# zhong-yy/volpick

Measured on AMD Instinct MI355X. Metric: waveform-windows/sec, higher is better.
Workload: dtype f32 (exact 3xbf16 split products, fp32 accumulate)

## Files before the change

volpick_amd/csrc/conv_b3.h:

```cpp
#pragma once
#include "bf16.h"
#include "conv_lds.h"

namespace vp {

typedef __bf16 bf16x8_b3 __attribute__((ext_vector_type(8)));

template <int C>
struct B3Image {
  static constexpr int CS = C + 8;
  bf16_t* img;
  int ps, c0;
};

__device__ __forceinline__ void b3_split(const float v, unsigned short& h, unsigned short& m, unsigned short& l) {
  h = to_bf16(v);
  const float r1 = v - from_bf16(h);
  m = to_bf16(r1);
  l = to_bf16(r1 - from_bf16(m));
}
__device__ __forceinline__ void b3_store4(bf16_t* img, const int ps, const int cs, const int col, const int ch, const float (&v)[4]) {
  const unsigned h0 = pack_bf16x2(v[0], v[1]), h1 = pack_bf16x2(v[2], v[3]);
  const float r0 = v[0] - bf16_lo(h0), r1 = v[1] - bf16_hi(h0), r2 = v[2] - bf16_lo(h1), r3 = v[3] - bf16_hi(h1);
  const unsigned m0 = pack_bf16x2(r0, r1), m1 = pack_bf16x2(r2, r3);
// ... 245 lines not shown
template <int C, int NC>
__device__ void b3c_dump(const bf16_t* img, const int c0, const int L, float* dst, const long ls, const int tid, const int nth) {
  using Q = B3Chunk<C, NC>;
  for (int k = tid; k < C * L; k += nth) {
    const int c = k / L, t = k - c * L;
    const bf16_t* p = img + (c >> 3) * Q::CHS + (t + c0) * 8 + (c & 7);
    dst[c * ls + t] = from_bf16(p[0]) + (from_bf16(p[Q::PS]) + from_bf16(p[2 * Q::PS]));
  }
}
#ifndef B3_EXP
#define B3_EXP 0
#endif
template <int C, int NC>
__device__ __forceinline__ void b3c_store4(bf16_t* img, const int col, const int quad, const float (&v)[4]) {
  using Q = B3Chunk<C, NC>;
  if (B3_EXP & 16) {
    asm volatile("" ::"v"(v[0]), "v"(v[1]), "v"(v[2]), "v"(v[3]));
    return;
  }
  const unsigned h0 = pack_bf16x2(v[0], v[1]), h1 = pack_bf16x2(v[2], v[3]);
  const float r0 = v[0] - bf16_lo(h0), r1 = v[1] - bf16_hi(h0), r2 = v[2] - bf16_lo(h1), r3 = v[3] - bf16_hi(h1);
  const unsigned m0 = pack_bf16x2(r0, r1), m1 = pack_bf16x2(r2, r3);
  const unsigned l0 = pack_bf16x2(r0 - bf16_lo(m0), r1 - bf16_hi(m0)), l1 = pack_bf16x2(r2 - bf16_lo(m1), r3 - bf16_hi(m1));
  bf16_t* p = img + (quad >> 1) * Q::CHS + col * 8 + (quad & 1) * 4;
  if (B3_EXP & 32) p = img + (quad >> 1) * Q::CHS + ((col >> 5) * 16 + (threadIdx.x & 15)) * 4;
  if (B3_EXP & 4) {
    asm volatile("" ::"v"(h0), "v"(h1), "v"(m0), "v"(m1), "v"(l0), "v"(l1), "v"(p));
    return;
  }
  *reinterpret_cast<uint2*>(p) = make_uint2(h0, h1);
  *reinterpret_cast<uint2*>(p + Q::PS) = make_uint2(m0, m1);
  *reinterpret_cast<uint2*>(p + 2 * Q::PS) = make_uint2(l0, l1);
}
template <int C, int NC, int TAPS>
__device__ __forceinline__ const bf16_t* b3c_lane_ptr(const bf16_t* img, const int col0, const int lane) {
  using G = B3Steps<C, TAPS>;
  const int g = lane >> 4;
  return img + (G::ch_of_lane(g) / 8) * B3Chunk<C, NC>::CHS + (col0 + (lane & 15) + G::tap_of_lane(g)) * 8;
}
struct B3NoSlot {
  __device__ __forceinline__ void operator()(int) const {}
};
template <int C, int NC, int TAPS, int NB, class Finish, class Slot = B3NoSlot>
__device__ __forceinline__ void b3c_mac_tiles(const bf16_t* p, const uint4 (&a)[B3Steps<C, TAPS>::STEPS * 3], Finish finish, Slot slot = Slot()) {
  using G = B3Steps<C, TAPS>;
  using Q = B3Chunk<C, NC>;
  constexpr int STEPS = G::STEPS;
  constexpr int AHEAD = 2, NBUF = AHEAD + 1, PAIRS = STEPS * NB;
  uint4 b[NBUF][3];
  auto load_b = [&](const int i) {
    const int s = i % STEPS, j = i / STEPS;
    const int off = ((C >= 32 ? s / G::KS : s * G::TPK) + j * 16) * 8 + (C >= 32 ? (s % G::KS) * 4 * Q::CHS : 0);
#pragma unroll
    for (int pc = 0; pc < 3; ++pc) b[i % NBUF][pc] = *reinterpret_cast<const uint4*>(p + pc * Q::PS + off);
  };
#pragma unroll
  for (int i = 0; i < AHEAD && i < PAIRS; ++i) load_b(i);
  f32x4 prev = {0.f, 0.f, 0.f, 0.f};
#pragma unroll
  for (int j = 0; j < NB; ++j) {
    f32x4 acc = {0.f, 0.f, 0.f, 0.f};
    __builtin_amdgcn_sched_barrier(0);
    if (j > 0) finish(j - 1, prev);
#pragma unroll
    for (int s = 0; s < STEPS; ++s) {
      const int i = j * STEPS + s;
// ... 27 lines not shown
      for (int pc = 0; pc < 3; ++pc) b[i & 1][h][pc] = *reinterpret_cast<const uint4*>(p + pc * Q::PS + off);
    }
  };
  load_b(0);
  f32x4 prev0 = {0.f, 0.f, 0.f, 0.f}, prev1 = prev0;
#pragma unroll
  for (int jp = 0; jp < NB / 2; ++jp) {
    f32x4 acc0 = {0.f, 0.f, 0.f, 0.f}, acc1 = acc0;
    __builtin_amdgcn_sched_barrier(0);
    if (jp > 0) {
      finish(2 * jp - 2, prev0);
      finish(2 * jp - 1, prev1);
    }
#pragma unroll
    for (int s = 0; s < STEPS; ++s) {
      const int i = jp * STEPS + s;
      if (i + 1 < PAIRS) load_b(i + 1);
      slot(i);
      constexpr int WP[6] = {2, 1, 0, 1, 0, 0}, XP[6] = {0, 1, 2, 0, 1, 0};
#pragma unroll
      for (int t = 0; t < 6; ++t) {
        acc0 = __builtin_amdgcn_mfma_f32_16x16x32_bf16(__builtin_bit_cast(bf16x8_b3, a[s * 3 + WP[t]]),
                                                      __builtin_bit_cast(bf16x8_b3, b[i & 1][0][XP[t]]), acc0, 0, 0, 0);
        acc1 = __builtin_amdgcn_mfma_f32_16x16x32_bf16(__builtin_bit_cast(bf16x8_b3, a[s * 3 + WP[t]]),
                                                      __builtin_bit_cast(bf16x8_b3, b[i & 1][1][XP[t]]), acc1, 0, 0, 0);
      }
    }
    __builtin_amdgcn_sched_barrier(0);
    prev0 = acc0;
    prev1 = acc1;
  }
  finish(NB - 2, prev0);
  finish(NB - 1, prev1);
}

template <int C, int NC, int TAPS, int NB>
__device__ __forceinline__ void b3c_mac_tiles_acc(const bf16_t* p, const uint4 (&a)[B3Steps<C, TAPS>::STEPS * 3], f32x4 (&acc)[NB]) {
  using G = B3Steps<C, TAPS>;
  using Q = B3Chunk<C, NC>;
  constexpr int STEPS = G::STEPS;
  constexpr int AHEAD = 1, NBUF = AHEAD + 1, PAIRS = STEPS * NB;
  uint4 b[NBUF][3];
  auto load_b = [&](const int i) {
    const int s = i % STEPS, j = i / STEPS;
    const int off = ((C >= 32 ? s / G::KS : s * G::TPK) + j * 16) * 8 + (C >= 32 ? (s % G::KS) * 4 * Q::CHS : 0);
#pragma unroll
    for (int pc = 0; pc < 3; ++pc) b[i % NBUF][pc] = *reinterpret_cast<const uint4*>(p + pc * Q::PS + off);
  };
  load_b(0);
#pragma unroll
  for (int j = 0; j < NB; ++j) {
#pragma unroll
    for (int s = 0; s < STEPS; ++s) {
      const int i = j * STEPS + s;
      if (i + AHEAD < PAIRS) load_b(i + AHEAD);
      __builtin_amdgcn_sched_barrier(0);
      constexpr int WP[6] = {2, 1, 0, 1, 0, 0}, XP[6] = {0, 1, 2, 0, 1, 0};
#pragma unroll
      for (int t = 0; t < 6; ++t)
        acc[j] = __builtin_amdgcn_mfma_f32_16x16x32_bf16(__builtin_bit_cast(bf16x8_b3, a[s * 3 + WP[t]]),
                                                        __builtin_bit_cast(bf16x8_b3, b[i % NBUF][XP[t]]), acc[j], 0, 0, 0);
      __builtin_amdgcn_sched_barrier(0);
    }
  }
}

// ... 72 lines not shown
```

volpick_amd/csrc/eqt_dec03.hip:

```cpp
#include <type_traits>

#include "conv_b3.h"
#include "conv_lds.h"
#include "eqt_kernels.h"
#include "net.h"

namespace vp {

namespace {

constexpr int D03_NTH = 512, D03_WAVES = 8;
using D_0 = LdsLayer<16, 0, 64, 2, 3, 1, -1, 0, 3, 1>;
using D_1 = LdsLayer<64, 0, 64, 2, 3, 1, -1, 0, 6, 1>;
using D_2 = LdsLayer<64, 0, 32, 2, 3, 1, -1, 0, 6, 1>;
using D_3 = LdsLayer<32, 0, 32, 2, 5, 1, -2, 0, 6, 1>;
constexpr int L0 = 47, L1 = 94, L2 = 188, L3 = 375, L4 = 750;
constexpr int C0 = 48, C1 = 96, C2 = 192, C3 = 384;
constexpr int S0 = 80, S1 = 112, S2 = 208, S3 = 400, BI = 4;
static_assert(S0 >= BI + C0 + 1 && S1 >= BI + 2 * C0 + 1 && S1 >= BI + C1 + 1 && S2 >= BI + 2 * C1 + 1 && S2 >= BI + C2 + 1 &&
                  S3 >= BI + 2 * C2 + 2 && S3 >= BI + C3 + 2,
              "image widths");
static_assert(S0 % 32 == 16 && S1 % 32 == 16 && S2 % 32 == 16 && S3 % 32 == 16, "bank-conflict-free strides");
constexpr int OFF0 = 0, OFF1 = OFF0 + 16 * S0, OFF2 = OFF1 + 64 * S1, OFF3 = OFF2 + 64 * S2, D03_LDS_FLOATS = OFF3 + 32 * S3;
static_assert(D03_LDS_FLOATS * 4 <= 160 * 1024 && OFF1 % 4 == 0 && OFF2 % 4 == 0 && OFF3 % 4 == 0, "LDS budget");

constexpr int B3_X1_NC = 112, B3_X2_NC = 208;
using QX1 = B3Chunk<64, B3_X1_NC>;
using QX2 = B3Chunk<64, B3_X2_NC>;
constexpr int B3_X1_PS = QX1::PS, B3_X2_PS = QX2::PS;
static_assert(B3_X1_NC >= C1 + 3 && B3_X2_NC >= C2 + 3, "every column stages 1 / 2 read has a place");
constexpr int B3_OFF_X2 = 0, B3_OFF_R = 3 * B3_X2_PS * 2;
constexpr int B3_OFF_X0 = B3_OFF_R, B3_OFF_X1 = B3_OFF_X0 + 16 * S0 * 4, B3_OFF_X3 = B3_OFF_R;
constexpr int B3_X3_NC = 400, B3_X3_C0 = 2;
using QX3 = B3Chunk<32, B3_X3_NC>;
constexpr int B3_OFF_EDGE = B3_OFF_X3 + 3 * QX3::PS * 2;
constexpr int B3_LDS_BYTES = B3_OFF_EDGE + D03_WAVES * 64 * 4;
static_assert(B3_X3_NC >= C3 + 4 + 0 && B3_X3_NC >= L3 + B3_X3_C0, "every column stage 3 reads has a place");
static_assert(B3_OFF_X1 + 3 * B3_X1_PS * 2 <= B3_LDS_BYTES && B3_LDS_BYTES <= 160 * 1024 && B3_OFF_R % 16 == 0 && B3_OFF_X1 % 16 == 0,
              "LDS budget of the bf16-piece variant");

struct Dec03Args {
  const float* x;
  int ls_x;
  long ws_x;
  float* y;
  int ls_y;
  long ws_y;
  const float* af[4];
  const float* bs[4];
  long af_stride[4];
  const uint4* af3[3];
  long af3_stride[3];
  const float* edge_w;
  const float* edge_b;
  int B, n_rows;
  int even_split;
  unsigned long long* clk;
};
struct Dec03DumpArgs : Dec03Args {
  float* dbg[3];
  int dbg_ls[3];
  long dbg_ws[3];
};

template <int S>
struct RowStore {
  float* img;
  unsigned len;
  __device__ __forceinline__ void operator()(int co, int t, float v) const { img[co * S + t] = ((unsigned)t < len) ? v : 0.f; }
  __device__ __forceinline__ bool all_valid(int t0, int t1) const { return (unsigned)t1 < len; }
// ... 27 lines not shown
          *reinterpret_cast<float2*>(row + t) =
              make_float2(fmaxf(acc[j][rr] + biasv[rr], 0.f), fmaxf(acc[j][rr + 1] + biasv[rr + 1], 0.f));
      }
    }
  }
};

struct Stage0Pieces {
  static constexpr bool custom_block_epilogue = true;
  bf16_t* img;
  __device__ __forceinline__ void quad(const int co, const int t, const float (&v)[4]) const {
    const float z[4] = {t < L1 ? v[0] : 0.f, t < L1 ? v[1] : 0.f, t < L1 ? v[2] : 0.f, t < L1 ? v[3] : 0.f};
    b3c_store4<64, B3_X1_NC>(img, t + 1, co >> 2, z);
  }
  template <class L>
  __device__ __forceinline__ void block_epilogue(const f32x4 (&acc)[L::NB], const float (&biasv)[4], const int mt, const int colb,
                                                 const int g, const int n) const {
    static_assert(L::P == 2 && L::RELU == 1 && L::OUT_OFF == 0 && L::COUT == 64, "stage 0 of the decoder");
#pragma unroll
    for (int j = 0; j < L::NB; ++j) {
      float v[4];
#pragma unroll
      for (int r = 0; r < 4; ++r) v[r] = fmaxf(acc[j][r] + biasv[r], 0.f);
      this->quad((mt & 3) * 16 + 4 * g, 2 * (colb + j * 16 + n) + (mt >> 2), v);
    }
  }
};
struct ClipQuad {
  bf16_t* img;
  int hi;
  __device__ __forceinline__ void quad(const int co, const int t, const float (&v)[4]) const {
    if (t < hi) b3c_store4<32, B3_X3_NC>(img, t + B3_X3_C0, co >> 2, v);
  }
};

template <bool B3, bool DUMP = false>
__global__ __launch_bounds__(D03_NTH) void eqt_dec03_kernel(const std::conditional_t<DUMP, Dec03DumpArgs, Dec03Args> a) {
  static_assert(!DUMP || B3, "DUMP instances exist for the default form only");
  extern __shared__ float4 d03_lds_raw[];
  float* lds = reinterpret_cast<float*>(d03_lds_raw);
  if constexpr (B3) {
    char* base = reinterpret_cast<char*>(d03_lds_raw);
    int o_r = B3_OFF_R / 16;
    asm volatile("" : "+v"(o_r));
    float* X0 = reinterpret_cast<float*>(base + 16 * o_r);
    bf16_t* X3 = reinterpret_cast<bf16_t*>(base + 16 * o_r);
    float* EDGE = reinterpret_cast<float*>(base + B3_OFF_EDGE);
    bf16_t* const X1 = reinterpret_cast<bf16_t*>(base + B3_OFF_X1);
    bf16_t* const X2 = reinterpret_cast<bf16_t*>(base + B3_OFF_X2);
    const int tid = threadIdx.x, lane = tid & 63, g = lane >> 4;
    const int wave_u = __builtin_amdgcn_readfirstlane(tid >> 6);
    int row = blockIdx.x;
    if (row >= a.n_rows) return;
    for (int i = tid; i < B3_LDS_BYTES / 16; i += D03_NTH) d03_lds_raw[i] = make_float4(0.f, 0.f, 0.f, 0.f);
    float pre[3];
    auto request = [&](int r) {
      const float* src = a.x + (long)r * a.ws_x + HALO;
#pragma unroll
      for (int k = 0; k < 3; ++k) {
        const int idx = tid + k * D03_NTH, c = idx / S0, t = idx - c * S0 - BI;
        pre[k] = (idx < 16 * S0 && (unsigned)t < (unsigned)L0) ? src[(long)c * a.ls_x + t] : 0.f;
      }
    };
    auto park = [&]() {
#pragma unroll
      for (int k = 0; k < 3; ++k) {
// ... 18 lines not shown
#if D3_CLOCK
    unsigned long long* clk = (a.clk && (tid & 255) == 0 && blockIdx.x == 0) ? a.clk + (tid >> 8) * 128 : nullptr;
    int stamp = 0;
#define D3_STAMP() \
  if (clk && stamp < 120) clk[stamp++] = __builtin_readcyclecounter();
#else
#define D3_STAMP()
#endif
    while (true) {
      const int next = row + gridDim.x;
      const bool more = next < a.n_rows;
      const int nd = more ? next / a.B : d;
      D3_STAMP()
      park();
      __syncthreads();
      D3_STAMP()
      uint4 a1[B3Steps<64, 3>::STEPS * 3];
      b3_load_a<64, 3>(a.af3[0] + d * a.af3_stride[0], wave_u, lane, a1);
      {
        Stage0Pieces st{X1};
        b3c_zero_rest<64, B3_X1_NC>(X1, 1, 1 + 2 * C0, tid, D03_NTH);
        conv_lds_areg<D_0, S0, BI, S0, BI>(X0, X0, areg0, bias0, wave_u, C0, st, 0, 1, lane);
      }
      const int n = lane & 15;
      {
        const int ph = wave_u >> 2, co0 = (wave_u & 3) * 16 + 4 * g;
        float bias1[4];
#pragma unroll
        for (int r = 0; r < 4; ++r) bias1[r] = a.bs[1][d * 64 + co0 + r];
        D3_STAMP()
        __syncthreads();
        D3_STAMP()
        if constexpr (DUMP) b3c_dump<64, B3_X1_NC>(X1, 1, L1, a.dbg[0] + (long)row * a.dbg_ws[0] + HALO, a.dbg_ls[0], tid, D03_NTH);
        b3c_mac_tile_pairs<64, B3_X1_NC, 3, 6>(b3c_lane_ptr<64, B3_X1_NC, 3>(X1, 0, lane), a1, [&](const int j, const f32x4 acc) {
          const int t = 2 * (j * 16 + n) + ph;
          float v[4];
#pragma unroll
          for (int r = 0; r < 4; ++r) v[r] = t < L2 ? fmaxf(acc[r] + bias1[r], 0.f) : 0.f;
          b3c_store4<64, B3_X2_NC>(X2, t + 1, co0 >> 2, v);
        });
      }
      D3_STAMP()
      uint4 a2[B3Steps<64, 3>::STEPS * 3];
      b3_load_a<64, 3>(a.af3[1] + d * a.af3_stride[1], wave_u & 3, lane, a2);
      __syncthreads();
      D3_STAMP()
      if constexpr (DUMP) b3c_dump<64, B3_X2_NC>(X2, 1, L2, a.dbg[1] + (long)row * a.dbg_ws[1] + HALO, a.dbg_ls[1], tid, D03_NTH);
      float eb;
      {
        constexpr int PADC = B3_X3_C0 + (B3_X3_NC - L3 - B3_X3_C0);
        if (tid < PADC * 12) {
          const int k = tid % PADC, cp = tid / PADC;
          const int col = k < B3_X3_C0 ? k : L3 + k;
          *reinterpret_cast<uint4*>(X3 + (cp >> 2) * QX3::PS + (cp & 3) * QX3::CHS + col * 8) = make_uint4(0u, 0u, 0u, 0u);
        }
        constexpr int n0 = (L3 - 2 - 2) >> 1;
        struct F3 {
          float x, y, z;
        };
        F3 ew[8];
        eb = a.edge_b[d * 32 + (lane >> 1)];
        const F3* e = reinterpret_cast<const F3*>(a.edge_w + ((long)d * 64 * 64 + lane) * 3 + (long)(8 * wave_u) * 64 * 3);
        const ClipQuad st{X3, L3 - 2};
        {
          const int mt2 = wave_u & 3, ph = mt2 >> 1, co0 = (mt2 & 1) * 16 + 4 * g, colb = (wave_u >> 2) * 96;
          float bias2[4];
#pragma unroll
          for (int r = 0; r < 4; ++r) bias2[r] = a.bs[2][d * 32 + co0 + r];
          b3c_mac_tile_pairs<64, B3_X2_NC, 3, 6>(b3c_lane_ptr<64, B3_X2_NC, 3>(X2, colb, lane), a2, [&](const int j, const f32x4 acc) {
            float v[4];
#pragma unroll
            for (int r = 0; r < 4; ++r) v[r] = fmaxf(acc[r] + bias2[r], 0.f);
            st.quad(co0, 2 * (colb + j * 16 + n) + ph, v);
            if constexpr (DUMP) {
              const int t = 2 * (colb + j * 16 + n) + ph;
              if (t < L3 - 2) {
                float* p = a.dbg[2] + (long)row * a.dbg_ws[2] + HALO + (long)co0 * a.dbg_ls[2] + t;
#pragma unroll
                for (int r = 0; r < 4; ++r) p[(long)r * a.dbg_ls[2]] = v[r];
              }
            }
          }, [&](const int i) {
            if (i % 2 == 0 && i / 2 < 8) ew[i / 2] = e[(i / 2) * 64];
          });
        }
        D3_STAMP()
        float pacc = 0.f;
        {
          float xk[3][8];
#pragma unroll
          for (int k = 0; k < 3; ++k) {
            uint4 q[3];
#pragma unroll
            for (int pc = 0; pc < 3; ++pc) q[pc] = *reinterpret_cast<const uint4*>(X2 + pc * QX2::PS + wave_u * QX2::CHS + (n0 + 1 + k) * 8);
            const unsigned* qh = reinterpret_cast<const unsigned*>(&q[0]);
            const unsigned* qm = reinterpret_cast<const unsigned*>(&q[1]);
            const unsigned* ql = reinterpret_cast<const unsigned*>(&q[2]);
#pragma unroll
            for (int i = 0; i < 4; ++i) {
              xk[k][2 * i] = (bf16_lo(qh[i]) + bf16_lo(qm[i])) + bf16_lo(ql[i]);
              xk[k][2 * i + 1] = (bf16_hi(qh[i]) + bf16_hi(qm[i])) + bf16_hi(ql[i]);
            }
          }
#pragma unroll
          for (int u = 0; u < 8; ++u) {
            pacc = fmaf(ew[u].x, xk[0][u], pacc);
            pacc = fmaf(ew[u].y, xk[1][u], pacc);
            pacc = fmaf(ew[u].z, xk[2][u], pacc);
          }
        }
        EDGE[wave_u * 64 + lane] = pacc;
      }
      D3_STAMP()
      uint4 a3[B3Steps<32, 5>::STEPS * 3];
      float bias3[4];
      b3_load_a<32, 5>(a.af3[2] + d * a.af3_stride[2], mt23, lane, a3);
#pragma unroll
      for (int r = 0; r < 4; ++r) bias3[r] = a.bs[3][d * 32 + mt23 * 8 + 2 * g + (r >> 1)];
      request(more ? next : row);
      load_stage0(nd);
      __syncthreads();
      D3_STAMP()
      if (blk23 == 1) {
        float acc = eb;
#pragma unroll
        for (int w8 = 0; w8 < D03_WAVES; ++w8) acc += EDGE[w8 * 64 + lane];
        unsigned short h, m, l;
        b3_split(fmaxf(acc, 0.f), h, m, l);
        const int ch = lane >> 1;
        bf16_t* q = X3 + (ch >> 3) * QX3::CHS + (L3 - 2 + (lane & 1) + B3_X3_C0) * 8 + (ch & 7);
        q[0] = h, q[QX3::PS] = m, q[2 * QX3::PS] = l;
        if constexpr (DUMP) {
          if (wave_u == 4) a.dbg[2][(long)row * a.dbg_ws[2] + HALO + (long)ch * a.dbg_ls[2] + L3 - 2 + (lane & 1)] = fmaxf(acc, 0.f);
        }
      }
      {
        float* yrow = a.y + (long)row * a.ws_y + HALO + (long)(mt23 * 8 + 2 * g) * a.ls_y;
        asm volatile("" ::"v"(bias3[0]), "v"(bias3[1]), "v"(bias3[2]), "v"(bias3[3]));
        auto stage3 = [&](const int colb, auto nb_tag) {
          constexpr int NB = decltype(nb_tag)::value;
          b3c_mac_tiles<32, B3_X3_NC, 5, NB>(b3c_lane_ptr<32, B3_X3_NC, 5>(X3, colb, lane), a3, [&](const int j, const f32x4 acc) {
            const int t = 2 * (colb + j * 16 + (lane & 15));
            if (t < L4) {
              *reinterpret_cast<float2*>(yrow + t) = make_float2(fmaxf(acc[0] + bias3[0], 0.f), fmaxf(acc[1] + bias3[1], 0.f));
              *reinterpret_cast<float2*>(yrow + a.ls_y + t) = make_float2(fmaxf(acc[2] + bias3[2], 0.f), fmaxf(acc[3] + bias3[3], 0.f));
            }
          });
        };
        if (a.even_split) {
          stage3(blk23 * 96, std::integral_constant<int, 6>{});
          stage3((blk23 + 2) * 96, std::integral_constant<int, 6>{});
        } else if (blk23 == 0) {
          stage3(0, std::integral_constant<int, 7>{});
          stage3(112, std::integral_constant<int, 7>{});
        } else {
          stage3(224, std::integral_constant<int, 5>{});
          stage3(304, std::integral_constant<int, 5>{});
        }
      }
      D3_STAMP()
      if (!more) break;
      row = next;
      d = nd;
      __syncthreads();
    }
#undef D3_STAMP
    return;
  }
  int off1 = OFF1 / 4, off2 = OFF2 / 4, off3 = OFF3 / 4;
  asm volatile("" : "+v"(off1), "+v"(off2), "+v"(off3));
  float* X0 = lds + OFF0;
  float* X1 = lds + 4 * off1;
  float* X2 = lds + 4 * off2;
  float* X3 = lds + 4 * off3;
  const int tid = threadIdx.x, lane = tid & 63;
  const int wave_u = __builtin_amdgcn_readfirstlane(tid >> 6);
  int row = blockIdx.x;
  if (row >= a.n_rows) return;
// ... 165 lines not shown
```

volpick_amd/csrc/eqt_tail_b3.hip:

```cpp
#include <type_traits>

#include "conv_b3.h"
#include "eqt_kernels.h"
#include "net.h"

namespace vp {

namespace {

constexpr int T_OUT = 6000;
constexpr int T3_NTH = 512, T3_WAVES = 8;
constexpr int HSB = 81, OUT_QS = 16 * HSB, OUT_PS = 2 * OUT_QS;
constexpr int HT_N = 43;
template <int TW_>
struct T3 {
  static constexpr int TW = TW_;
  static constexpr int NB4O = 3, NB4Y = TW_ > 1200 ? 3 : 2, NB5 = 5, NB6 = 5;
  static constexpr int C4 = 2 * (NB4O + NB4Y) * 16, C5 = 4 * NB5 * 16, C6 = T3_WAVES * NB6 * 16;
  static constexpr int PARK_COLS = TW_ > 1200 ? 176 : 168;
  static constexpr int NC4 = 208, NC5 = (2 * C4 > C5 + 16 ? 2 * C4 : C5 + 16), NC6 = C6 + 16;
  static constexpr int BLOCKS = (TW_ + 15) / 16;
  using Q4 = B3Chunk<32, NC4>;
  using Q5 = B3Chunk<16, NC5>;
  using Q6 = B3Chunk<16, NC6>;
  static constexpr bool GUARD5 = 2 * C5 > NC6;
  static constexpr bool ZERO6 = (TW_ + 12) / 2 + 7 >= 2 * C5;
  static constexpr int R0_BYTES = 3 * Q6::PS * 2, R1_BYTES = 3 * OUT_PS * 8;
  static constexpr int A5_N = 2 * B3Steps<16, 5>::STEPS * 3 * 64, A6_N = B3Steps<16, 7>::STEPS * 3 * 64;
  static constexpr int OFF_R1 = R0_BYTES, OFF_HT = OFF_R1 + R1_BYTES, OFF_A5 = OFF_HT + 3 * HT_N * 16 + 48, OFF_A6 = OFF_A5 + A5_N * 16;
  static constexpr int LDS_BYTES = OFF_A6 + A6_N * 16;
  static_assert(OFF_A5 % 16 == 0, "16-byte fragments");
  static_assert(3 * Q4::PS * 2 <= R0_BYTES && 3 * Q5::PS * 2 <= R1_BYTES && LDS_BYTES <= 160 * 1024 && OFF_R1 % 16 == 0 && OFF_HT % 16 == 0,
                "LDS budget");
  static_assert(NC4 >= PARK_COLS && NC5 >= C5 + 6 && NC6 >= C6 + 8 && NC5 >= 2 * C4 && (GUARD5 || NC6 >= 2 * C5) && HSB % 2 == 1,
                "every column a stage reads or writes has a place");
  static_assert(TW % 8 == 0, "tile grid: 16-byte stores of the heads, whole stage-3 samples");
  static_assert(TW + 11 <= 2 * C6 && C6 / 8 <= HSB - 1 && (BLOCKS + 15) / 16 <= T3_WAVES, "stage 6 / heads");
  static_assert((TW + 12) / 2 + 7 < NC6 && (!ZERO6 || 2 * C5 % 2 == 0), "the padded taps of stage 6 stay inside its input image");
  static_assert(TW / 2 + 6 + 6 <= 2 * C5 && TW / 2 + 6 + 6 <= NC6 && TW / 4 + 6 + 5 <= 2 * C4 && TW / 8 + 6 + 4 <= PARK_COLS, "halo chain");
  static_assert(((((TW + 12) / 2 + 7) / 2 + 1 + 5) / 2 + 4) < PARK_COLS, "closure of the kept outputs under the padded taps");
  static_assert(PARK_COLS * 8 <= 3 * T3_NTH && PARK_COLS * 8 > 2 * T3_NTH, "three (four channels x one sample) items per thread");
  static constexpr double GROUPS = 4.0 * (NB4O + NB4Y) * 5 + 8.0 * NB5 * 3 + 8.0 * NB6 * 4 + 5.0 * 7;
};

struct Tail3Args {
  const float* x3;
  int ls3;
  long ws3;
  float* y;
  const uint4 *af4, *af5, *af6;
  long af4_stride, af5_stride, af6_stride;
  const float *bs4, *bs5, *bs6;
  const uint4* head_t;
  const float* head_b;
  const float* flags;
  int B, n_tiles;
  int t_lo, tiles_per_row;
  unsigned long long* clk;
};
struct Tail3DumpArgs : Tail3Args {
  float* dbg[4];
  int dbg_ls[4];
  long dbg_ws[4];
};

struct Tile3 {
  int d, win, t0;
};
template <int TW>
__device__ __forceinline__ Tile3 tile3_id(const int tile, const Tail3Args& a) {
  const int row = tile / a.tiles_per_row, j = tile - row * a.tiles_per_row;
  return Tile3{row / a.B, row, a.t_lo + j * TW};
}

__device__ __forceinline__ void t3_finish(const f32x4 acc, const float (&bias)[4], const bool in, float (&v)[4]) {
#pragma unroll
  for (int r = 0; r < 4; ++r) v[r] = in ? fmaxf(acc[r] + bias[r], 0.f) : 0.f;
}

template <int TW_, bool DUMP = false>
__global__ __launch_bounds__(T3_NTH) void eqt_tail3_kernel(const std::conditional_t<DUMP, Tail3DumpArgs, Tail3Args> a) {
  static_assert(!DUMP || TW_ == 1200, "DUMP instances exist for the 1200-sample tiling only");
  using K = T3<TW_>;
  using Q5 = typename K::Q5;
  using Q6 = typename K::Q6;
  constexpr int TW = K::TW, NB4O = K::NB4O, NB4Y = K::NB4Y, NB5 = K::NB5, NB6 = K::NB6, PARK_COLS = K::PARK_COLS, NC4 = K::NC4,
                NC5 = K::NC5, NC6 = K::NC6, C5 = K::C5, BLOCKS = K::BLOCKS, OFF_R1 = K::OFF_R1, OFF_HT = K::OFF_HT, OFF_A5 = K::OFF_A5, OFF_A6 = K::OFF_A6,
                A5_N = K::A5_N, A6_N = K::A6_N, T3_LDS_BYTES = K::LDS_BYTES;
  (void)sizeof(Q5), (void)sizeof(Q6);
  extern __shared__ uint4 t3_lds[];
  char* base = reinterpret_cast<char*>(t3_lds);
  bf16_t* IN4 = reinterpret_cast<bf16_t*>(base);
  bf16_t* IN6 = IN4;
  bf16_t* IN5 = reinterpret_cast<bf16_t*>(base + OFF_R1);
  uint2* OUT6 = reinterpret_cast<uint2*>(base + OFF_R1);
  uint4* HT = reinterpret_cast<uint4*>(base + OFF_HT);
  uint4* A5 = reinterpret_cast<uint4*>(base + OFF_A5);
  uint4* A6 = reinterpret_cast<uint4*>(base + OFF_A6);
  const int tid = threadIdx.x, lane = tid & 63, n = lane & 15, g = lane >> 4;
  const int w = __builtin_amdgcn_readfirstlane(tid >> 6);
  int tile = blockIdx.x;
  if (tile >= a.n_tiles) return;
  for (int i = tid; i < T3_LDS_BYTES / 16; i += T3_NTH) t3_lds[i] = make_uint4(0u, 0u, 0u, 0u);
  Tile3 id = tile3_id<TW>(tile, a);
  unsigned long long* clk = (a.clk && tid == 0 && (int)blockIdx.x < a.B) ? a.clk + (long)blockIdx.x * 32 : nullptr;
  int n_done = 0;
  auto dump = [&](const int i, const int co, const int s, const int lo, const int len, const float (&v)[4]) {
    if constexpr (DUMP) {
      if ((unsigned)(s - lo) < (unsigned)len) {
        float* p = a.dbg[i] + (long)id.win * a.dbg_ws[i] + HALO + (long)co * a.dbg_ls[i] + s;
// ... 39 lines not shown

  uint4 a4[B3Steps<32, 5>::STEPS * 3];
  float bias4[4], bias5[4], bias6[4], bh;
  auto load_weights = [&](const int d) {
    b3_load_a<32, 5>(a.af4 + d * a.af4_stride, w & 1, lane, a4);
    for (int i = tid; i < A5_N; i += T3_NTH) A5[i] = a.af5[d * a.af5_stride + i];
    for (int i = tid; i < A6_N; i += T3_NTH) A6[i] = a.af6[d * a.af6_stride + i];
#pragma unroll
    for (int r = 0; r < 4; ++r) {
      bias4[r] = a.bs4[d * 16 + 4 * g + r];
      bias5[r] = a.bs5[d * 16 + 4 * g + r];
      bias6[r] = a.bs6[d * 8 + 4 * (g & 1) + r];
    }
    bh = a.head_b[d];
    if (tid < 3 * HT_N) HT[tid] = a.head_t[d * 3 * HT_N + tid];
  };
  __syncthreads();
  load_weights(id.d);

  while (true) {
    const int next = tile + gridDim.x;
    const bool more = next < a.n_tiles;
    const Tile3 nid = more ? tile3_id<TW>(next, a) : id;
    const int t0 = id.t0;
    const float win_flag = a.flags ? a.flags[id.win - id.d * a.B] : 0.f;
    T3_STAMP(0)
    park();
    __syncthreads();
    T3_STAMP(1)
    {
      const bool older = w < 4;
      const int ph = w & 1, colb = older ? (w >> 1) * (NB4O * 16) : 2 * NB4O * 16 + ((w - 4) >> 1) * (NB4Y * 16);
      const int lo = 6 - t0 / 4;
      auto finish = [&](const int j, const f32x4 acc) {
        const int t = 2 * (colb + j * 16 + n) + ph;
        float v[4];
        t3_finish(acc, bias4, (unsigned)(t - lo) < 1500u, v);
        b3c_store4<16, NC5>(IN5, t, g, v);
        if constexpr (DUMP) dump(0, 4 * g, t0 / 4 - 6 + t, t0 / 4, TW / 4, v);
      };
      if (older) b3c_mac_tiles<32, NC4, 5, NB4O>(b3c_lane_ptr<32, NC4, 5>(IN4, colb, lane), a4, finish);
      else b3c_mac_tiles<32, NC4, 5, NB4Y>(b3c_lane_ptr<32, NC4, 5>(IN4, colb, lane), a4, finish);
    }
    __syncthreads();
    T3_STAMP(2)
    {
      const int ph = w & 1, colb = (w >> 1) * (NB5 * 16);
      uint4 a5[B3Steps<16, 5>::STEPS * 3];
#pragma unroll
      for (int i = 0; i < B3Steps<16, 5>::STEPS * 3; ++i) a5[i] = A5[ph * (A5_N / 2) + i * 64 + lane];
      const int lo = 6 - t0 / 2;
      auto finish = [&](const int j, const f32x4 acc) {
        const int t = 2 * (colb + j * 16 + n) + ph;
        float v[4];
        t3_finish(acc, bias5, (unsigned)(t - lo) < 3000u, v);
        if (!K::GUARD5 || t < NC6) b3c_store4<16, NC6>(IN6, t, g, v);
        if constexpr (DUMP) dump(1, 4 * g, t0 / 2 - 6 + t, t0 / 2, TW / 2, v);
      };
      if (K::ZERO6) {
        constexpr int ZC = NC6 - 2 * C5, UNITS = 3 * 2 * ZC;
        for (int i = tid; i < UNITS; i += T3_NTH) {
          const int plane = i / ZC, col = 2 * C5 + (i - plane * ZC);
          *reinterpret_cast<uint4*>(IN6 + (plane >> 1) * Q6::PS + (plane & 1) * Q6::CHS + col * 8) = make_uint4(0u, 0u, 0u, 0u);
        }
      }
      b3c_mac_tiles<16, NC5, 5, NB5>(b3c_lane_ptr<16, NC5, 5>(IN5, colb + 1, lane), a5, finish);
    }
    __syncthreads();
    T3_STAMP(3)
    {
      const int colb = w * (NB6 * 16), ph = g >> 1;
      uint4 a6[B3Steps<16, 7>::STEPS * 3];
#pragma unroll
      for (int i = 0; i < B3Steps<16, 7>::STEPS * 3; ++i) a6[i] = A6[i * 64 + lane];
      const int lo = 6 - t0;
      uint2* q = OUT6 + (g & 1) * OUT_QS + ((2 * n + ph) & 15) * HSB + (n >> 3) + colb / 8;
      auto finish = [&](const int j, const f32x4 acc) {
        const int t = 2 * (colb + j * 16 + n) + ph;
        float v[4];
        t3_finish(acc, bias6, (unsigned)(t - lo) < (unsigned)T_OUT, v);
        if constexpr (DUMP) dump(2, 4 * (g & 1), t0 - 6 + t, t0, TW, v);
        if (B3_EXP & 16) {
          asm volatile("" ::"v"(v[0]), "v"(v[1]), "v"(v[2]), "v"(v[3]));
          return;
        }
        const unsigned h0 = pack_bf16x2(v[0], v[1]), h1 = pack_bf16x2(v[2], v[3]);
        const float r0 = v[0] - bf16_lo(h0), r1 = v[1] - bf16_hi(h0), r2 = v[2] - bf16_lo(h1), r3 = v[3] - bf16_hi(h1);
        const unsigned m0 = pack_bf16x2(r0, r1), m1 = pack_bf16x2(r2, r3);
        const unsigned l0 = pack_bf16x2(r0 - bf16_lo(m0), r1 - bf16_hi(m0)), l1 = pack_bf16x2(r2 - bf16_lo(m1), r3 - bf16_hi(m1));
        if (B3_EXP & 4) {
          asm volatile("" ::"v"(h0), "v"(h1), "v"(m0), "v"(m1), "v"(l0), "v"(l1), "v"(q));
          return;
        }
        q[2 * j] = make_uint2(h0, h1);
        q[2 * j + OUT_PS] = make_uint2(m0, m1);
        q[2 * j + 2 * OUT_PS] = make_uint2(l0, l1);
      };
      b3c_mac_tiles<16, NC6, 7, NB6>(b3c_lane_ptr<16, NC6, 7>(IN6, colb, lane), a6, finish, [&](const int i) {
        if (i < 12) request_part(nid, i);
      });
    }
    __syncthreads();
    T3_STAMP(4)
    if (w < (BLOCKS + 15) / 16) {
      f32x4 acc = {bh, bh, bh, bh};
      const uint2* bp = OUT6 + (16 * w + n);
      const uint4* ap = HT + (g - n + 15);
      constexpr int HD = 1, HB = HD + 1;
      uint4 av[HB][3], bv[HB][3];
      auto load_ab = [&](const int s, uint4 (&aa)[3], uint4 (&bb)[3]) {
        const int e = 4 * s + g + 1, chunk = (e & 15) * HSB + (e >> 4);
#pragma unroll
        for (int pc = 0; pc < 3; ++pc) {
          aa[pc] = ap[pc * HT_N + 4 * s];
          const uint2 c0 = bp[pc * OUT_PS + chunk], c1 = bp[pc * OUT_PS + OUT_QS + chunk];
          bb[pc] = make_uint4(c0.x, c0.y, c1.x, c1.y);
        }
      };
#pragma unroll
      for (int s = 0; s < HD && s < 7; ++s) load_ab(s, av[s % HB], bv[s % HB]);
#pragma unroll
      for (int s = 0; s < 7; ++s) {
        if (s + HD < 7) load_ab(s + HD, av[(s + HD) % HB], bv[(s + HD) % HB]);
        __builtin_amdgcn_sched_barrier(0);
        constexpr int WP[6] = {2, 1, 0, 1, 0, 0}, XP[6] = {0, 1, 2, 0, 1, 0};
#pragma unroll
        for (int t = 0; t < 6; ++t)
          acc = __builtin_amdgcn_mfma_f32_16x16x32_bf16(__builtin_bit_cast(bf16x8_b3, av[s % HB][WP[t]]),
                                                       __builtin_bit_cast(bf16x8_b3, bv[s % HB][XP[t]]), acc, 0, 0, 0);
        __builtin_amdgcn_sched_barrier(0);
      }
// ... 125 lines not shown
```

Measured before the change: 3.464 million.

## Slice 3xbf16 epilogue across K-steps and overlap weight reads with barriers

Splits each tile's epilogue (bias/relu, then hi/mid/lo bf16 split and store) into three parts. Each part runs during one of the next tile's K-steps, with sched_group_barrier interleaving MFMAs and the VALU/LDS work, so the epilogue hides under matrix math instead of stalling after each tile. In the tail kernel, the next stage's weight fragments are read from LDS before a custom s_waitcnt+s_barrier that leaves those reads outstanding. Store addresses are precomputed once per stage. This raises register pressure and makes correctness depend on hand-written waitcnt counts and on schedule hints.

After: 3.455 million, median of 2. Within noise of the previous version (-0.3%).

```diff
diff --git a/volpick_amd/csrc/conv_b3.h b/volpick_amd/csrc/conv_b3.h
--- a/volpick_amd/csrc/conv_b3.h
+++ b/volpick_amd/csrc/conv_b3.h
@@ -301,6 +301,60 @@
   *reinterpret_cast<uint2*>(p + Q::PS) = make_uint2(m0, m1);
   *reinterpret_cast<uint2*>(p + 2 * Q::PS) = make_uint2(l0, l1);
 }
+#ifndef B3C_SLICED
+#define B3C_SLICED 1
+#endif
+struct B3cSplit {
+  float v[4];
+  unsigned p0, p1;
+};
+template <int C, int NC>
+__device__ __forceinline__ bf16_t* b3c_quad_ptr(bf16_t* img, const int col, const int quad) {
+  using Q = B3Chunk<C, NC>;
+  if (B3_EXP & 32) return img + (quad >> 1) * Q::CHS + ((col >> 5) * 16 + (threadIdx.x & 15)) * 4;
+  return img + (quad >> 1) * Q::CHS + col * 8 + (quad & 1) * 4;
+}
+template <int C, int NC>
+__device__ __forceinline__ void b3c_store_piece(bf16_t* p, const int pc, const unsigned d0, const unsigned d1) {
+  if (B3_EXP & 4) {
+    asm volatile("" ::"v"(d0), "v"(d1), "v"(p));
+    return;
+  }
+  *reinterpret_cast<uint2*>(p + pc * B3Chunk<C, NC>::PS) = make_uint2(d0, d1);
+}
+template <class Values, class Store>
+struct B3cFinish {
+  using State = B3cSplit;
+  Values values;
+  Store store;
+  __device__ __forceinline__ void a(const int j, const f32x4 acc, State& s) const {
+    values(j, acc, s.v);
+    if (B3_EXP & 16) {
+      asm volatile("" ::"v"(s.v[0]), "v"(s.v[1]), "v"(s.v[2]), "v"(s.v[3]));
+      return;
+    }
+    s.p0 = pack_bf16x2(s.v[0], s.v[1]), s.p1 = pack_bf16x2(s.v[2], s.v[3]);
+    store(j, 0, s.p0, s.p1);
+  }
+  __device__ __forceinline__ void b(const int j, State& s) const {
+    if (B3_EXP & 16) return;
+    s.v[0] -= bf16_lo(s.p0), s.v[1] -= bf16_hi(s.p0), s.v[2] -= bf16_lo(s.p1), s.v[3] -= bf16_hi(s.p1);
+    s.p0 = pack_bf16x2(s.v[0], s.v[1]), s.p1 = pack_bf16x2(s.v[2], s.v[3]);
+    store(j, 1, s.p0, s.p1);
+  }
+  __device__ __forceinline__ void c(const int j, State& s) const {
+    if (B3_EXP & 16) return;
+    store(j, 2, pack_bf16x2(s.v[0] - bf16_lo(s.p0), s.v[1] - bf16_hi(s.p0)), pack_bf16x2(s.v[2] - bf16_lo(s.p1), s.v[3] - bf16_hi(s.p1)));
+  }
+  __device__ __forceinline__ void operator()(const int j, const f32x4 acc) const {
+    State s;
+    a(j, acc, s), b(j, s), c(j, s);
+  }
+};
+template <class Values, class Store>
+__device__ __forceinline__ B3cFinish<Values, Store> b3c_finish(Values values, Store store) {
+  return B3cFinish<Values, Store>{values, store};
+}
 template <int C, int NC, int TAPS>
 __device__ __forceinline__ const bf16_t* b3c_lane_ptr(const bf16_t* img, const int col0, const int lane) {
   using G = B3Steps<C, TAPS>;
@@ -394,6 +448,127 @@
   }
   finish(NB - 2, prev0);
   finish(NB - 1, prev1);
+}
+
+template <int MFMAS, int PER>
+__device__ __forceinline__ void b3c_spread() {
+#pragma unroll
+  for (int t = 0; t < MFMAS; ++t) {
+    __builtin_amdgcn_sched_group_barrier(0x008, 1, 0);
+    __builtin_amdgcn_sched_group_barrier(0x002 | 0x200, PER, 0);
+  }
+}
+template <int C, int NC, int TAPS, int NB, class Fin, class Slot = B3NoSlot>
+__device__ __forceinline__ void b3c_mac_tiles_sliced(const bf16_t* p, const uint4 (&a)[B3Steps<C, TAPS>::STEPS * 3], Fin fin, Slot slot = Slot()) {
+#if !B3C_SLICED
+  b3c_mac_tiles<C, NC, TAPS, NB>(p, a, fin, slot);
+#else
+  using G = B3Steps<C, TAPS>;
+  using Q = B3Chunk<C, NC>;
+  constexpr int STEPS = G::STEPS;
+  static_assert(STEPS >= 3, "three parts need three K-steps");
+  constexpr int AHEAD = 1, NBUF = AHEAD + 1, PAIRS = STEPS * NB;
+  uint4 b[NBUF][3];
+  auto load_b = [&](const int i) {
+    const int s = i % STEPS, j = i / STEPS;
+    const int off = ((C >= 32 ? s / G::KS : s * G::TPK) + j * 16) * 8 + (C >= 32 ? (s % G::KS) * 4 * Q::CHS : 0);
+#pragma unroll
+    for (int pc = 0; pc < 3; ++pc) b[i % NBUF][pc] = *reinterpret_cast<const uint4*>(p + pc * Q::PS + off);
+  };
+#pragma unroll
+  for (int i = 0; i < AHEAD && i < PAIRS; ++i) load_b(i);
+  f32x4 prev = {0.f, 0.f, 0.f, 0.f};
+  typename Fin::State st;
+#pragma unroll
+  for (int j = 0; j < NB; ++j) {
+    f32x4 acc = {0.f, 0.f, 0.f, 0.f};
+#pragma unroll
+    for (int s = 0; s < STEPS; ++s) {
+      const int i = j * STEPS + s;
+      __builtin_amdgcn_sched_barrier(0);
+      if (i + AHEAD < PAIRS) load_b(i + AHEAD);
+      slot(i);
+      if (j > 0 && s == 0) fin.a(j - 1, prev, st);
+      if (j > 0 && s == 1) fin.b(j - 1, st);
+      if (j > 0 && s == 2) fin.c(j - 1, st);
+      constexpr int WP[6] = {2, 1, 0, 1, 0, 0}, XP[6] = {0, 1, 2, 0, 1, 0};
+#pragma unroll
+      for (int t = 0; t < 6; ++t)
+        acc = __builtin_amdgcn_mfma_f32_16x16x32_bf16(__builtin_bit_cast(bf16x8_b3, a[s * 3 + WP[t]]),
+                                                     __builtin_bit_cast(bf16x8_b3, b[i % NBUF][XP[t]]), acc, 0, 0, 0);
+      if (j > 0 && s < 3) b3c_spread<6, 3>();
+    }
+    __builtin_amdgcn_sched_barrier(0);
+    prev = acc;
+  }
+  fin.a(NB - 1, prev, st);
+  fin.b(NB - 1, st);
+  fin.c(NB - 1, st);
+#endif
+}
+template <int C, int NC, int TAPS, int NB, class Fin, class Slot = B3NoSlot>
+__device__ __forceinline__ void b3c_mac_tile_pairs_sliced(const bf16_t* p, const uint4 (&a)[B3Steps<C, TAPS>::STEPS * 3], Fin fin, Slot slot = Slot()) {
+#if !B3C_SLICED
+  b3c_mac_tile_pairs<C, NC, TAPS, NB>(p, a, fin, slot);
+#else
+  using G = B3Steps<C, TAPS>;
+  using Q = B3Chunk<C, NC>;
+  static_assert(NB % 2 == 0, "pairs of n-tiles");
+  constexpr int STEPS = G::STEPS, PAIRS = STEPS * (NB / 2);
+  static_assert(STEPS >= 3, "three parts need three K-steps");
+  constexpr bool STAGGER = STEPS >= 6;
+  uint4 b[2][2][3];
+  auto load_b = [&](const int i) {
+    const int s = i % STEPS, jp = i / STEPS;
+#pragma unroll
+    for (int h = 0; h < 2; ++h) {
+      const int off = ((C >= 32 ? s / G::KS : s * G::TPK) + (2 * jp + h) * 16) * 8 + (C >= 32 ? (s % G::KS) * 4 * Q::CHS : 0);
+#pragma unroll
+      for (int pc = 0; pc < 3; ++pc) b[i & 1][h][pc] = *reinterpret_cast<const uint4*>(p + pc * Q::PS + off);
+    }
+  };
+  load_b(0);
+  f32x4 prev0 = {0.f, 0.f, 0.f, 0.f}, prev1 = prev0;
+  typename Fin::State st0, st1;
+#pragma unroll
+  for (int jp = 0; jp < NB / 2; ++jp) {
+    f32x4 acc0 = {0.f, 0.f, 0.f, 0.f}, acc1 = acc0;
+#pragma unroll
+    for (int s = 0; s < STEPS; ++s) {
+      const int i = jp * STEPS + s;
+      __builtin_amdgcn_sched_barrier(0);
+      if (i + 1 < PAIRS) load_b(i + 1);
+      slot(i);
+      if (STAGGER) {
+        if (jp > 0 && s == 0) fin.a(2 * jp - 2, prev0, st0);
+        if (jp > 0 && s == 1) fin.b(2 * jp - 2, st0);
+        if (jp > 0 && s == 2) fin.c(2 * jp - 2, st0);
+        if (jp > 0 && s == 3) fin.a(2 * jp - 1, prev1, st0);
+        if (jp > 0 && s == 4) fin.b(2 * jp - 1, st0);
+        if (jp > 0 && s == 5) fin.c(2 * jp - 1, st0);
+      } else {
+        if (jp > 0 && s == 0) fin.a(2 * jp - 2, prev0, st0), fin.a(2 * jp - 1, prev1, st1);
+        if (jp > 0 && s == 1) fin.b(2 * jp - 2, st0), fin.b(2 * jp - 1, st1);
+        if (jp > 0 && s == 2) fin.c(2 * jp - 2, st0), fin.c(2 * jp - 1, st1);
+      }
+      constexpr int WP[6] = {2, 1, 0, 1, 0, 0}, XP[6] = {0, 1, 2, 0, 1, 0};
+#pragma unroll
+      for (int t = 0; t < 6; ++t) {
+        acc0 = __builtin_amdgcn_mfma_f32_16x16x32_bf16(__builtin_bit_cast(bf16x8_b3, a[s * 3 + WP[t]]),
+                                                      __builtin_bit_cast(bf16x8_b3, b[i & 1][0][XP[t]]), acc0, 0, 0, 0);
+        acc1 = __builtin_amdgcn_mfma_f32_16x16x32_bf16(__builtin_bit_cast(bf16x8_b3, a[s * 3 + WP[t]]),
+                                                      __builtin_bit_cast(bf16x8_b3, b[i & 1][1][XP[t]]), acc1, 0, 0, 0);
+      }
+      if (jp > 0 && s < (STAGGER ? 6 : 3)) b3c_spread<12, STAGGER ? 2 : 3>();
+    }
+    __builtin_amdgcn_sched_barrier(0);
+    prev0 = acc0;
+    prev1 = acc1;
+  }
+  fin.a(NB - 2, prev0, st0), fin.a(NB - 1, prev1, st1);
+  fin.b(NB - 2, st0), fin.b(NB - 1, st1);
+  fin.c(NB - 2, st0), fin.c(NB - 1, st1);
+#endif
 }
 
 template <int C, int NC, int TAPS, int NB>
diff --git a/volpick_amd/csrc/eqt_dec03.hip b/volpick_amd/csrc/eqt_dec03.hip
--- a/volpick_amd/csrc/eqt_dec03.hip
+++ b/volpick_amd/csrc/eqt_dec03.hip
@@ -36,6 +36,7 @@
 constexpr int B3_OFF_EDGE = B3_OFF_X3 + 3 * QX3::PS * 2;
 constexpr int B3_LDS_BYTES = B3_OFF_EDGE + D03_WAVES * 64 * 4;
 static_assert(B3_X3_NC >= C3 + 4 + 0 && B3_X3_NC >= L3 + B3_X3_C0, "every column stage 3 reads has a place");
+static_assert(B3_X3_NC >= 2 * C2 + B3_X3_C0, "every column stage 2 computes has a place (ClipQuad::first)");
 static_assert(B3_OFF_X1 + 3 * B3_X1_PS * 2 <= B3_LDS_BYTES && B3_LDS_BYTES <= 160 * 1024 && B3_OFF_R % 16 == 0 && B3_OFF_X1 % 16 == 0,
               "LDS budget of the bf16-piece variant");
 
@@ -129,6 +130,8 @@
   __device__ __forceinline__ void quad(const int co, const int t, const float (&v)[4]) const {
     if (t < hi) b3c_store4<32, B3_X3_NC>(img, t + B3_X3_C0, co >> 2, v);
   }
+  __device__ __forceinline__ bool keeps(const int t) const { return t < hi; }
+  __device__ __forceinline__ bf16_t* first(const int co, const int t) const { return b3c_quad_ptr<32, B3_X3_NC>(img, t + B3_X3_C0, co >> 2); }
 };
 
 template <bool B3, bool DUMP = false>
@@ -213,13 +216,21 @@
         __syncthreads();
         D3_STAMP()
         if constexpr (DUMP) b3c_dump<64, B3_X1_NC>(X1, 1, L1, a.dbg[0] + (long)row * a.dbg_ws[0] + HALO, a.dbg_ls[0], tid, D03_NTH);
-        b3c_mac_tile_pairs<64, B3_X1_NC, 3, 6>(b3c_lane_ptr<64, B3_X1_NC, 3>(X1, 0, lane), a1, [&](const int j, const f32x4 acc) {
-          const int t = 2 * (j * 16 + n) + ph;
-          float v[4];
-#pragma unroll
-          for (int r = 0; r < 4; ++r) v[r] = t < L2 ? fmaxf(acc[r] + bias1[r], 0.f) : 0.f;
-          b3c_store4<64, B3_X2_NC>(X2, t + 1, co0 >> 2, v);
-        });
+        bf16_t* const out1 = b3c_quad_ptr<64, B3_X2_NC>(X2, 2 * n + ph + 1, co0 >> 2);
+        b3c_mac_tile_pairs_sliced<64, B3_X1_NC, 3, 6>(
+            b3c_lane_ptr<64, B3_X1_NC, 3>(X1, 0, lane), a1,
+            b3c_finish(
+                [&](const int j, const f32x4 acc, float (&v)[4]) {
+                  const int t = 2 * (j * 16 + n) + ph;
+#pragma unroll
+                  for (int r = 0; r < 4; ++r) {
+                    const float x = fmaxf(acc[r] + bias1[r], 0.f);
+                    v[r] = t < L2 ? x : 0.f;
+                  }
+                },
+                [&](const int j, const int pc, const unsigned d0, const unsigned d1) {
+                  b3c_store_piece<64, B3_X2_NC>(out1 + j * (32 * 8), pc, d0, d1);
+                }));
       }
       D3_STAMP()
       uint4 a2[B3Steps<64, 3>::STEPS * 3];
@@ -248,22 +259,31 @@
           float bias2[4];
 #pragma unroll
           for (int r = 0; r < 4; ++r) bias2[r] = a.bs[2][d * 32 + co0 + r];
-          b3c_mac_tile_pairs<64, B3_X2_NC, 3, 6>(b3c_lane_ptr<64, B3_X2_NC, 3>(X2, colb, lane), a2, [&](const int j, const f32x4 acc) {
-            float v[4];
-#pragma unroll
-            for (int r = 0; r < 4; ++r) v[r] = fmaxf(acc[r] + bias2[r], 0.f);
-            st.quad(co0, 2 * (colb + j * 16 + n) + ph, v);
-            if constexpr (DUMP) {
-              const int t = 2 * (colb + j * 16 + n) + ph;
-              if (t < L3 - 2) {
-                float* p = a.dbg[2] + (long)row * a.dbg_ws[2] + HALO + (long)co0 * a.dbg_ls[2] + t;
-#pragma unroll
-                for (int r = 0; r < 4; ++r) p[(long)r * a.dbg_ls[2]] = v[r];
-              }
-            }
-          }, [&](const int i) {
-            if (i % 2 == 0 && i / 2 < 8) ew[i / 2] = e[(i / 2) * 64];
-          });
+          bf16_t* const out2 = st.first(co0, 2 * (colb + n) + ph);
+          b3c_mac_tile_pairs_sliced<64, B3_X2_NC, 3, 6>(
+              b3c_lane_ptr<64, B3_X2_NC, 3>(X2, colb, lane), a2,
+              b3c_finish(
+                  [&](const int j, const f32x4 acc, float (&v)[4]) {
+                    const int t = 2 * (colb + j * 16 + n) + ph;
+#pragma unroll
+                    for (int r = 0; r < 4; ++r) {
+                      const float x = fmaxf(acc[r] + bias2[r], 0.f);
+                      v[r] = st.keeps(t) ? x : 0.f;
+                    }
+                    if constexpr (DUMP) {
+                      if (t < L3 - 2) {
+                        float* p = a.dbg[2] + (long)row * a.dbg_ws[2] + HALO + (long)co0 * a.dbg_ls[2] + t;
+#pragma unroll
+                        for (int r = 0; r < 4; ++r) p[(long)r * a.dbg_ls[2]] = v[r];
+                      }
+                    }
+                  },
+                  [&](const int j, const int pc, const unsigned d0, const unsigned d1) {
+                    b3c_store_piece<32, B3_X3_NC>(out2 + j * (32 * 8), pc, d0, d1);
+                  }),
+              [&](const int i) {
+                if (i % 2 == 0 && i / 2 < 8) ew[i / 2] = e[(i / 2) * 64];
+              });
         }
         D3_STAMP()
         float pacc = 0.f;
@@ -320,11 +340,12 @@
         asm volatile("" ::"v"(bias3[0]), "v"(bias3[1]), "v"(bias3[2]), "v"(bias3[3]));
         auto stage3 = [&](const int colb, auto nb_tag) {
           constexpr int NB = decltype(nb_tag)::value;
+          float* const y0 = yrow + 2 * (colb + (lane & 15));
           b3c_mac_tiles<32, B3_X3_NC, 5, NB>(b3c_lane_ptr<32, B3_X3_NC, 5>(X3, colb, lane), a3, [&](const int j, const f32x4 acc) {
             const int t = 2 * (colb + j * 16 + (lane & 15));
             if (t < L4) {
-              *reinterpret_cast<float2*>(yrow + t) = make_float2(fmaxf(acc[0] + bias3[0], 0.f), fmaxf(acc[1] + bias3[1], 0.f));
-              *reinterpret_cast<float2*>(yrow + a.ls_y + t) = make_float2(fmaxf(acc[2] + bias3[2], 0.f), fmaxf(acc[3] + bias3[3], 0.f));
+              *reinterpret_cast<float2*>(y0 + 32 * j) = make_float2(fmaxf(acc[0] + bias3[0], 0.f), fmaxf(acc[1] + bias3[1], 0.f));
+              *reinterpret_cast<float2*>(y0 + a.ls_y + 32 * j) = make_float2(fmaxf(acc[2] + bias3[2], 0.f), fmaxf(acc[3] + bias3[3], 0.f));
             }
           });
         };
diff --git a/volpick_amd/csrc/eqt_tail_b3.hip b/volpick_amd/csrc/eqt_tail_b3.hip
--- a/volpick_amd/csrc/eqt_tail_b3.hip
+++ b/volpick_amd/csrc/eqt_tail_b3.hip
@@ -34,6 +34,7 @@
                 "LDS budget");
   static_assert(NC4 >= PARK_COLS && NC5 >= C5 + 6 && NC6 >= C6 + 8 && NC5 >= 2 * C4 && (GUARD5 || NC6 >= 2 * C5) && HSB % 2 == 1,
                 "every column a stage reads or writes has a place");
+  static_assert(!GUARD5, "a guarded store is a branch in stage 5's sliced epilogue: see b3c_mac_tiles_sliced before using such a tiling");
   static_assert(TW % 8 == 0, "tile grid: 16-byte stores of the heads, whole stage-3 samples");
   static_assert(TW + 11 <= 2 * C6 && C6 / 8 <= HSB - 1 && (BLOCKS + 15) / 16 <= T3_WAVES, "stage 6 / heads");
   static_assert((TW + 12) / 2 + 7 < NC6 && (!ZERO6 || 2 * C5 % 2 == 0), "the padded taps of stage 6 stay inside its input image");
@@ -73,9 +74,18 @@
   return Tile3{row / a.B, row, a.t_lo + j * TW};
 }
 
+template <int KEEP>
+__device__ __forceinline__ void t3_barrier_keep() {
+  static_assert(KEEP >= 0 && KEEP <= 15, "lgkmcnt is a four-bit counter");
+  asm volatile("s_waitcnt lgkmcnt(%0)\n\ts_barrier" ::"n"(KEEP) : "memory");
+}
+
 __device__ __forceinline__ void t3_finish(const f32x4 acc, const float (&bias)[4], const bool in, float (&v)[4]) {
 #pragma unroll
-  for (int r = 0; r < 4; ++r) v[r] = in ? fmaxf(acc[r] + bias[r], 0.f) : 0.f;
+  for (int r = 0; r < 4; ++r) {
+    const float x = fmaxf(acc[r] + bias[r], 0.f);
+    v[r] = in ? x : 0.f;
+  }
 }
 
 template <int TW_, bool DUMP = false>
@@ -181,31 +191,54 @@
       const bool older = w < 4;
       const int ph = w & 1, colb = older ? (w >> 1) * (NB4O * 16) : 2 * NB4O * 16 + ((w - 4) >> 1) * (NB4Y * 16);
       const int lo = 6 - t0 / 4;
-      auto finish = [&](const int j, const f32x4 acc) {
-        const int t = 2 * (colb + j * 16 + n) + ph;
-        float v[4];
-        t3_finish(acc, bias4, (unsigned)(t - lo) < 1500u, v);
-        b3c_store4<16, NC5>(IN5, t, g, v);
-        if constexpr (DUMP) dump(0, 4 * g, t0 / 4 - 6 + t, t0 / 4, TW / 4, v);
-      };
-      if (older) b3c_mac_tiles<32, NC4, 5, NB4O>(b3c_lane_ptr<32, NC4, 5>(IN4, colb, lane), a4, finish);
-      else b3c_mac_tiles<32, NC4, 5, NB4Y>(b3c_lane_ptr<32, NC4, 5>(IN4, colb, lane), a4, finish);
-    }
-    __syncthreads();
+      bf16_t* const out4 = b3c_quad_ptr<16, NC5>(IN5, 2 * (colb + n) + ph, g);
+      const auto finish = b3c_finish(
+          [&](const int j, const f32x4 acc, float (&v)[4]) {
+            const int t = 2 * (colb + j * 16 + n) + ph;
+            t3_finish(acc, bias4, (unsigned)(t - lo) < 1500u, v);
+            if constexpr (DUMP) dump(0, 4 * g, t0 / 4 - 6 + t, t0 / 4, TW / 4, v);
+          },
+          [&](const int j, const int pc, const unsigned d0, const unsigned d1) {
+            b3c_store_piece<16, NC5>(out4 + j * (32 * 8), pc, d0, d1);
+          });
+      if (older) b3c_mac_tiles_sliced<32, NC4, 5, NB4O>(b3c_lane_ptr<32, NC4, 5>(IN4, colb, lane), a4, finish);
+      else b3c_mac_tiles_sliced<32, NC4, 5, NB4Y>(b3c_lane_ptr<32, NC4, 5>(IN4, colb, lane), a4, finish);
+    }
+    uint4 a5[B3Steps<16, 5>::STEPS * 3], a6[B3Steps<16, 7>::STEPS * 3];
+    auto read_a5 = [&]() {
+      int o = OFF_A5 / 16 + (w & 1) * (A5_N / 2) + lane;
+      asm volatile("" : "+v"(o));
+#pragma unroll
+      for (int i = 0; i < B3Steps<16, 5>::STEPS * 3; ++i) a5[i] = t3_lds[o + i * 64];
+    };
+    auto read_a6 = [&]() {
+      int o = OFF_A6 / 16 + lane;
+      asm volatile("" : "+v"(o));
+#pragma unroll
+      for (int i = 0; i < B3Steps<16, 7>::STEPS * 3; ++i) a6[i] = t3_lds[o + i * 64];
+    };
+    if constexpr (B3C_SLICED != 0) {
+      __builtin_amdgcn_sched_barrier(0);
+      read_a5();
+      t3_barrier_keep<B3Steps<16, 5>::STEPS * 3>();
+    } else {
+      __syncthreads();
+      read_a5();
+    }
     T3_STAMP(2)
     {
       const int ph = w & 1, colb = (w >> 1) * (NB5 * 16);
-      uint4 a5[B3Steps<16, 5>::STEPS * 3];
-#pragma unroll
-      for (int i = 0; i < B3Steps<16, 5>::STEPS * 3; ++i) a5[i] = A5[ph * (A5_N / 2) + i * 64 + lane];
       const int lo = 6 - t0 / 2;
-      auto finish = [&](const int j, const f32x4 acc) {
-        const int t = 2 * (colb + j * 16 + n) + ph;
-        float v[4];
-        t3_finish(acc, bias5, (unsigned)(t - lo) < 3000u, v);
-        if (!K::GUARD5 || t < NC6) b3c_store4<16, NC6>(IN6, t, g, v);
-        if constexpr (DUMP) dump(1, 4 * g, t0 / 2 - 6 + t, t0 / 2, TW / 2, v);
-      };
+      bf16_t* const out5 = b3c_quad_ptr<16, NC6>(IN6, 2 * (colb + n) + ph, g);
+      const auto finish = b3c_finish(
+          [&](const int j, const f32x4 acc, float (&v)[4]) {
+            const int t = 2 * (colb + j * 16 + n) + ph;
+            t3_finish(acc, bias5, (unsigned)(t - lo) < 3000u, v);
+            if constexpr (DUMP) dump(1, 4 * g, t0 / 2 - 6 + t, t0 / 2, TW / 2, v);
+          },
+          [&](const int j, const int pc, const unsigned d0, const unsigned d1) {
+            if (!K::GUARD5 || 2 * (colb + j * 16 + n) + ph < NC6) b3c_store_piece<16, NC6>(out5 + j * (32 * 8), pc, d0, d1);
+          });
       if (K::ZERO6) {
         constexpr int ZC = NC6 - 2 * C5, UNITS = 3 * 2 * ZC;
         for (int i = tid; i < UNITS; i += T3_NTH) {
@@ -213,39 +246,35 @@
           *reinterpret_cast<uint4*>(IN6 + (plane >> 1) * Q6::PS + (plane & 1) * Q6::CHS + col * 8) = make_uint4(0u, 0u, 0u, 0u);
         }
       }
-      b3c_mac_tiles<16, NC5, 5, NB5>(b3c_lane_ptr<16, NC5, 5>(IN5, colb + 1, lane), a5, finish);
-    }
-    __syncthreads();
+      b3c_mac_tiles_sliced<16, NC5, 5, NB5>(b3c_lane_ptr<16, NC5, 5>(IN5, colb + 1, lane), a5, finish);
+    }
+    if constexpr (B3C_SLICED != 0) {
+      __builtin_amdgcn_sched_barrier(0);
+      read_a6();
+      t3_barrier_keep<B3Steps<16, 7>::STEPS * 3>();
+    } else {
+      __syncthreads();
+      read_a6();
+    }
     T3_STAMP(3)
     {
       const int colb = w * (NB6 * 16), ph = g >> 1;
-      uint4 a6[B3Steps<16, 7>::STEPS * 3];
-#pragma unroll
-      for (int i = 0; i < B3Steps<16, 7>::STEPS * 3; ++i) a6[i] = A6[i * 64 + lane];
       const int lo = 6 - t0;
       uint2* q = OUT6 + (g & 1) * OUT_QS + ((2 * n + ph) & 15) * HSB + (n >> 3) + colb / 8;
-      auto finish = [&](const int j, const f32x4 acc) {
-        const int t = 2 * (colb + j * 16 + n) + ph;
-        float v[4];
-        t3_finish(acc, bias6, (unsigned)(t - lo) < (unsigned)T_OUT, v);
-        if constexpr (DUMP) dump(2, 4 * (g & 1), t0 - 6 + t, t0, TW, v);
-        if (B3_EXP & 16) {
-          asm volatile("" ::"v"(v[0]), "v"(v[1]), "v"(v[2]), "v"(v[3]));
-          return;
-        }
-        const unsigned h0 = pack_bf16x2(v[0], v[1]), h1 = pack_bf16x2(v[2], v[3]);
-        const float r0 = v[0] - bf16_lo(h0), r1 = v[1] - bf16_hi(h0), r2 = v[2] - bf16_lo(h1), r3 = v[3] - bf16_hi(h1);
-        const unsigned m0 = pack_bf16x2(r0, r1), m1 = pack_bf16x2(r2, r3);
-        const unsigned l0 = pack_bf16x2(r0 - bf16_lo(m0), r1 - bf16_hi(m0)), l1 = pack_bf16x2(r2 - bf16_lo(m1), r3 - bf16_hi(m1));
-        if (B3_EXP & 4) {
-          asm volatile("" ::"v"(h0), "v"(h1), "v"(m0), "v"(m1), "v"(l0), "v"(l1), "v"(q));
-          return;
-        }
-        q[2 * j] = make_uint2(h0, h1);
-        q[2 * j + OUT_PS] = make_uint2(m0, m1);
-        q[2 * j + 2 * OUT_PS] = make_uint2(l0, l1);
-      };
-      b3c_mac_tiles<16, NC6, 7, NB6>(b3c_lane_ptr<16, NC6, 7>(IN6, colb, lane), a6, finish, [&](const int i) {
+      const auto finish = b3c_finish(
+          [&](const int j, const f32x4 acc, float (&v)[4]) {
+            const int t = 2 * (colb + j * 16 + n) + ph;
+            t3_finish(acc, bias6, (unsigned)(t - lo) < (unsigned)T_OUT, v);
+            if constexpr (DUMP) dump(2, 4 * (g & 1), t0 - 6 + t, t0, TW, v);
+          },
+          [&](const int j, const int pc, const unsigned d0, const unsigned d1) {
+            if (B3_EXP & 4) {
+              asm volatile("" ::"v"(d0), "v"(d1), "v"(q));
+              return;
+            }
+            q[2 * j + pc * OUT_PS] = make_uint2(d0, d1);
+          });
+      b3c_mac_tiles_sliced<16, NC6, 7, NB6>(b3c_lane_ptr<16, NC6, 7>(IN6, colb, lane), a6, finish, [&](const int i) {
         if (i < 12) request_part(nid, i);
       });
     }
```
